# ruanjue/smartdenovo

Measured on AMD Instinct MI355X. Metric: Gbp of candidate pairs aligned/sec (wtzmo all-vs-all), higher is better.
Workload: dtype int32/int16

## Files before the change

### smartdenovo_amd/csrc/wtz_stitch_fused.h

```cpp
#ifndef WTZ_STITCH_FUSED_H
#define WTZ_STITCH_FUSED_H

#include "wtz_tasks.h"
#include "wtz_sw_frame.h"
#include "wtz_sw_frame16.h"

#ifdef __HIPCC__
template<int TW>
__device__ __attribute__((noinline)) bool wtz_extjob_run_fr_call(wtz_extjob_t *job, const wtz_params_t *Pm, wtz_pool_t *pool, wtz_pool_t *tpool){
	__shared__ uint64_t stb[TW];
	return wtz_extjob_run_fr<TW>(job, Pm, pool, tpool, stb);
}
template<int TW>
__device__ __attribute__((noinline)) void wtz_stitch_mid_call(uint32_t t, const wtz_env_t *V, const wtz_alnitem_t *items, wtz_stitch_state_t *sts, const wtz_extjob_t *jobsL, wtz_extjob_t *jobsR, const wtz_gapres_t *gaps){
	wtz_task_stitch_mid(t, *V, items, sts, jobsL, jobsR, gaps, true);
}
template<int TW>
__global__ void __launch_bounds__(64) __attribute__((amdgpu_waves_per_eu(WTZ_OCC_EXTFR, 8))) wtz_kernel_stitch_ext_fr(const wtz_env_t V, const wtz_alnitem_t *items, wtz_stitch_state_t *sts,
		wtz_extjob_t *jobsL, wtz_extjob_t *jobsR, const wtz_gapres_t *gaps, const uint32_t *order, uint32_t n, uint32_t stride, uint32_t first){
	const uint32_t b = blockIdx.x;
	if(b >= n) return;
	const uint32_t t = order[(size_t)b * stride + first];
	#pragma nounroll
	for(int side = 0; side < 2; side++){
		if(side){
			wtz_stitch_mid_call<TW>(t, &V, items, sts, jobsL, jobsR, gaps);
			__threadfence_block();
		}
		if(!wtz_extjob_run_fr_call<TW>(side ? &jobsR[t] : &jobsL[t], V.P, V.pool, V.pool + 1)) return;
		__threadfence_block();
	}
}
#define WTZ_PK_LDS_BYTES(TW) ((TW) * 8 + 64)
template<int TW>
__device__ __attribute__((always_inline)) inline bool wtz_extjob_run_pk_call(wtz_extjob_t *job, const wtz_params_t *Pm, wtz_pool_t *pool, wtz_pool_t *tpool){
	return wtz_extjob_run_pk<TW>(job, Pm, pool, tpool, (uint64_t*)wtz_wave_scratch());
}
template<int TW>
__global__ void __launch_bounds__(64) __attribute__((amdgpu_waves_per_eu(WTZ_OCC_EXTPK, 8))) wtz_kernel_stitch_ext_pk(const wtz_env_t V, const wtz_alnitem_t *items, wtz_stitch_state_t *sts,
		wtz_extjob_t *jobsL, wtz_extjob_t *jobsR, const wtz_gapres_t *gaps, const uint32_t *order, uint32_t n, uint32_t stride, uint32_t first, uint32_t *open){
	const uint32_t b = blockIdx.x;
	if(b >= n) return;
	const uint32_t t = order[(size_t)b * stride + first];
	#pragma nounroll
	for(int side = 0; side < 2; side++){
		if(side){
			wtz_task_stitch_mid(t, V, items, sts, jobsL, jobsR, gaps, true);
			__threadfence_block();
		}
		if(!wtz_extjob_run_pk_call<TW>(side ? &jobsR[t] : &jobsL[t], V.P, V.pool, V.pool + 1)){
			if((threadIdx.x & 63u) == 0){ const uint32_t k = atomicAdd(&open[0], 1u); open[1 + k] = t; }
			return;
		}
		__threadfence_block();
	}
}
#endif

#endif
```

### smartdenovo_amd/csrc/wtz_sw_frame16.h

```cpp
#ifndef WTZ_SW_FRAME16_H
#define WTZ_SW_FRAME16_H

#include "wtz_sw_frame.h"

#ifdef __HIPCC__

#ifndef WTZ_OCC_EXTPK
#define WTZ_OCC_EXTPK 4
#endif

typedef short wtz_v2s __attribute__((ext_vector_type(2)));
WTZ_D uint32_t wtz_pk_max(uint32_t a, uint32_t b){ return __builtin_bit_cast(uint32_t, __builtin_elementwise_max(__builtin_bit_cast(wtz_v2s, a), __builtin_bit_cast(wtz_v2s, b))); }
WTZ_D uint32_t wtz_pk_adds(uint32_t a, uint32_t b){ return __builtin_bit_cast(uint32_t, __builtin_elementwise_add_sat(__builtin_bit_cast(wtz_v2s, a), __builtin_bit_cast(wtz_v2s, b))); }
WTZ_D uint32_t wtz_pk_subs(uint32_t a, uint32_t b){ return __builtin_bit_cast(uint32_t, __builtin_elementwise_sub_sat(__builtin_bit_cast(wtz_v2s, a), __builtin_bit_cast(wtz_v2s, b))); }
WTZ_D uint32_t wtz_pk_mad(uint32_t a, uint32_t b, uint32_t c){ uint32_t r; asm("v_pk_mad_u16 %0, %1, %2, %3" : "=v"(r) : "v"(a), "v"(b), "v"(c)); return r; }
WTZ_D uint32_t wtz_bfi(uint32_t mask, uint32_t a, uint32_t b){ uint32_t r; asm("v_bfi_b32 %0, %1, %2, %3" : "=v"(r) : "s"(mask), "v"(a), "v"(b)); return r; }
WTZ_D uint32_t wtz_pk2(int32_t lo, int32_t hi){ return ((uint32_t)lo & 0xFFFFu) | ((uint32_t)hi << 16); }
WTZ_D int32_t wtz_pk_lo(uint32_t a){ return (int32_t)(int16_t)(a & 0xFFFFu); }
WTZ_D int32_t wtz_pk_hi(uint32_t a){ return (int32_t)a >> 16; }
WTZ_D uint32_t wtz_pk_join(uint32_t hi, uint32_t lo){ return __builtin_amdgcn_alignbit(hi, lo, 16); }
template<int H>
WTZ_D uint32_t wtz_pk_eqacc(uint32_t acc, uint32_t v, uint32_t t){
	if constexpr(H) asm("v_cmp_eq_u16_sdwa vcc, %1, %2 src0_sel:WORD_1 src1_sel:WORD_0\n\tv_addc_co_u32_e32 %0, vcc, %0, %0, vcc" : "+v"(acc) : "v"(v), "v"(t) : "vcc");
	else asm("v_cmp_eq_u16_sdwa vcc, %1, %2 src0_sel:WORD_0 src1_sel:WORD_0\n\tv_addc_co_u32_e32 %0, vcc, %0, %0, vcc" : "+v"(acc) : "v"(v), "v"(t) : "vcc");
	return acc;
}
WTZ_D uint32_t wtz_even_bits(uint64_t x){
	x &= 0x5555555555555555ULL;
	x = (x | (x >> 1)) & 0x3333333333333333ULL; x = (x | (x >> 2)) & 0x0F0F0F0F0F0F0F0FULL; x = (x | (x >> 4)) & 0x00FF00FF00FF00FFULL;
	x = (x | (x >> 8)) & 0x0000FFFF0000FFFFULL; x = (x | (x >> 16)) & 0x00000000FFFFFFFFULL;
	return (uint32_t)x;
}

template<int C2, int S>
WTZ_D void wtz_pk_row(uint32_t (&hv)[C2], uint32_t (&ev)[C2], uint32_t (&zw)[(C2 + 3) / 4], uint32_t (&gm)[(C2 + 3) / 4], const uint32_t eqw, const uint32_t bndp, const uint32_t SFp,
		const int32_t SF, const int32_t O, const uint32_t MXp, const uint32_t Xpp, const uint32_t Op, const uint32_t (&ckp)[C2]){
	uint32_t agg = 0x80008000u;
	auto cell1 = [&](auto kc, const uint32_t src) -> uint32_t {
		constexpr int k = decltype(kc)::value;
		const uint32_t b = (k ? (eqw >> k) : eqw) & 0x00010001u;
		const uint32_t m = wtz_pk_adds(wtz_pk_mad(b, MXp, src), Xpp);
		agg = wtz_pk_max(agg, m);
		return m;
	};
	if constexpr(S == 0){
		const uint32_t prv = (uint32_t)wtz_dpp_wave_shr1((int32_t)bndp, (int32_t)hv[C2 - 1]);
		const uint32_t src0 = wtz_pk_join(hv[C2 - 1], prv);
		wtz_static_for<0, C2>([&](auto kc){
			constexpr int k = C2 - 1 - decltype(kc)::value;
			hv[k] = cell1(wtz_ic<k>{}, (k == 0) ? src0 : hv[k == 0 ? 0 : k - 1]);
		});
	} else if constexpr(S == 1){
		wtz_static_for<0, C2>([&](auto kc){ constexpr int k = decltype(kc)::value; hv[k] = cell1(kc, hv[k]); });
	} else {
		const uint32_t nxt = (uint32_t)wtz_dpp_wave_shl1((int32_t)SFp, (int32_t)hv[0]);
		const uint32_t srcl = wtz_pk_join(nxt, hv[0]);
		wtz_static_for<0, C2>([&](auto kc){
			constexpr int k = decltype(kc)::value;
			hv[k] = cell1(kc, (k == C2 - 1) ? srcl : hv[k == C2 - 1 ? k : k + 1]);
		});
	}
	uint32_t f;
	{
		const int32_t aA = wtz_pk_lo(agg), aB = wtz_pk_hi(agg);
		const int32_t aL = aA > aB ? aA : aB;
		const int32_t pm = wtz_wave_max_scan_excl(aL + O, SF);
		const int32_t fA = pm > SF ? pm : SF;
		const int32_t fB = fA > aA + O ? fA : aA + O;
		f = wtz_pk2(fA, fB);
	}
	uint32_t ne0 = 0, ne1 = 0;
	if constexpr(S >= 1) ne0 = wtz_pk_join((uint32_t)wtz_dpp_wave_shl1((int32_t)SFp, (int32_t)ev[0]), ev[0]);
	if constexpr(S == 2) ne1 = wtz_pk_join((uint32_t)wtz_dpp_wave_shl1((int32_t)SFp, (int32_t)ev[C2 > 1 ? 1 : 0]), ev[C2 > 1 ? 1 : 0]);
	wtz_static_for<0, C2>([&](auto kc){
		constexpr int k = decltype(kc)::value;
		const uint32_t m = hv[k];
		uint32_t e;
		if constexpr(S == 0) e = ev[k];
		else if constexpr(S == 1) e = (k == C2 - 1) ? ne0 : ev[k == C2 - 1 ? k : k + 1];
		else e = (k == C2 - 1) ? ne1 : ((k == C2 - 2) ? ne0 : ev[k >= C2 - 2 ? k : k + 2]);
		const uint32_t h0 = wtz_pk_max(m, e);
		const uint32_t s0 = wtz_pk_subs(m, e);
		const uint32_t s1 = wtz_pk_subs(h0, f);
		const uint32_t h = wtz_pk_max(h0, f);
		const uint32_t t = wtz_pk_adds(m, Op);
		const uint32_t s2 = wtz_pk_subs(t, e);
		const uint32_t en = wtz_pk_max(e, t);
		const uint32_t s3 = wtz_pk_subs(t, f);
		f = wtz_pk_max(f, t);
		hv[k] = h; ev[k] = en;
		const uint32_t x01 = wtz_bfi(0x80008000u, s0, s1 >> 1), x23 = wtz_bfi(0x80008000u, s2, s3 >> 1);
		const uint32_t x = wtz_bfi(0xC000C000u, x01, x23 >> 2);
		const uint32_t v = wtz_pk_adds(h, ckp[k]);
		if constexpr((k & 3) == 0){ gm[k >> 2] = v; zw[k >> 2] = x >> 12; }
		else {
			gm[k >> 2] = wtz_pk_max(gm[k >> 2], v);
			if constexpr((k & 3) == 1) zw[k >> 2] = wtz_bfi(0x00F000F0u, x >> 8, zw[k >> 2]);
			else if constexpr((k & 3) == 2) zw[k >> 2] = wtz_bfi(0x0F000F00u, x >> 4, zw[k >> 2]);
			else zw[k >> 2] = wtz_bfi(0xF000F000u, x, zw[k >> 2]);
		}
		if constexpr((k & 3) == 3 || k == C2 - 1){ WTZ_PIN(zw[k >> 2]); }
	});
}

template<int C2>
WTZ_D bool wtz_shift_traceback_pk(wtz_aln_t &x, uint8_t **zchunk, const int32_t *zb, uint32_t zrow, uint32_t *lds, wtz_cigar_t &cigars, const wtz_tb_score *sc){
	const int lane = (int)(threadIdx.x & 63);
	constexpr int C = 2 * C2, CQ = (C2 + 3) / 4, NL = 64;
	constexpr int NLW = (128 / C) < NL ? (128 / C) : NL;
	constexpr int NDW = NLW * CQ, ROWB = NLW * C;
	static_assert(NDW <= 64 && ROWB <= 128, "window geometry");
	uint32_t *S32 = lds; uint8_t *S8 = (uint8_t*)lds; uint8_t *Sd = S8 + 8192;
	int32_t i_ = x.qe, j_ = x.te; uint32_t d_ = 0;
#ifdef WTZ_EXP_NOTB
	i_ = -1; j_ = -1;
#endif
	uint32_t run_op = 0xFFu, run_len = 0;
	int32_t n_gap_runs = 0; bool consistent = true;
	wtz_cigw_t Wr; Wr.v = &cigars; Wr.tail = 0;
	int32_t cc = 0;
	if(i_ >= 0) cc = j_ - wtz_as_global(zb)[i_];
	const int ln_off = lane / CQ, q4 = lane % CQ;
	while(i_ >= 0 && j_ >= 0){
		const int32_t i0 = i_;
		int32_t L0 = (cc < 0 ? 0 : (cc > NL * C - 1 ? NL * C - 1 : cc)) / C - NLW / 2;
		if(L0 > NL - NLW) L0 = NL - NLW;
		if(L0 < 0) L0 = 0;
		const int32_t CC0 = L0 * C;
		{
			const int32_t r = i0 - lane;
			Sd[lane] = (r >= 1) ? (uint8_t)(wtz_as_global(zb)[r] - wtz_as_global(zb)[r - 1]) : (uint8_t)0;
		}
		const int32_t cA = i0 >> 6;
		const uint8_t *chA = wtz_as_global(zchunk)[cA];
		const uint8_t *chB = cA > 0 ? wtz_as_global(zchunk)[cA - 1] : chA;
		const bool act = lane < NDW && (L0 + ln_off) < NL;
		const uint32_t doff = act ? ((uint32_t)q4 * (uint32_t)NL + (uint32_t)(L0 + ln_off)) * 4u : 0u;
		const uint32_t pos0 = (uint32_t)ln_off * (uint32_t)C + (uint32_t)q4 * 4u;
		for(int r8 = 0; r8 < 64; r8 += 8){
			uint32_t w8[8];
			#pragma unroll
			for(int u = 0; u < 8; u++){
				int32_t r = i0 - (r8 + u); if(r < 0) r = 0;
				const uint8_t *rowp = ((r >> 6) == cA ? chA : chB) + (size_t)(r & 63) * zrow;
				w8[u] = *wtz_as_global((const uint32_t*)(rowp + doff));
			}
			if(act){
				#pragma unroll
				for(int u = 0; u < 8; u++){
					const uint32_t pos = (uint32_t)(r8 + u) * 128u + pos0;
					#pragma unroll
					for(int hh = 0; hh < 2; hh++){
						uint32_t w = hh ? (w8[u] >> 16) : (w8[u] & 0xFFFFu);
						w = (w | (w << 8)) & 0x00FF00FFu; w = (w | (w << 4)) & 0x0F0F0F0Fu;
						const uint32_t a = (w >> 2) & 0x01010101u, b = (w >> 3) & 0x01010101u;
						const uint32_t v = (a << 1) | (b & (a ^ 0x01010101u)) | ((w & 0x02020202u) << 1) | ((w & 0x01010101u) << 5);
						const uint32_t p = pos + (hh ? (uint32_t)C2 : 0u);
						if constexpr((C2 & 3) == 0) S32[p >> 2] = v;
						else {
							#pragma unroll
							for(int k = 0; k < 4; k++) if(q4 * 4 + k < C2) S8[p + k] = (uint8_t)(v >> (8 * k));
						}
					}
				}
			}
		}
		__threadfence_block();
		if(lane == 0){
			while(i_ >= 0 && j_ >= 0){
				const int32_t rr = i0 - i_;
				if(rr >= 64) break;
				uint32_t zv = 0;
				if((uint32_t)cc < (uint32_t)(NL * C)){
					const int32_t t = cc - CC0;
					if((uint32_t)t >= (uint32_t)ROWB) break;
					zv = S8[rr * 128 + t];
				}
				const int32_t sft = (int32_t)Sd[rr];
				d_ = (zv >> (d_ << 1)) & 0x03;
				if(d_ == 0){ x.mat++; i_--; j_--; cc += sft - 1; }
				else if(d_ == 1){ i_--; x.ins++; cc += sft; }
				else { j_--; x.del++; cc--; }
				if(d_ == run_op) run_len++;
				else { if(run_len) wtz_cigw_push(Wr, run_op, run_len); run_op = d_; run_len = 1; if(d_) n_gap_runs++; }
			}
		}
		i_ = __builtin_amdgcn_readfirstlane(i_); j_ = __builtin_amdgcn_readfirstlane(j_); cc = __builtin_amdgcn_readfirstlane(cc);
		__threadfence_block();
	}
	if(lane == 0){
		if(run_len) wtz_cigw_push(Wr, run_op, run_len);
		if(i_ >= 0){ x.ins += i_ + 1; wtz_cigw_push(Wr, 1, (uint32_t)(i_ + 1)); n_gap_runs++; }
		if(j_ >= 0){ x.del += j_ + 1; wtz_cigw_push(Wr, 2, (uint32_t)(j_ + 1)); n_gap_runs++; }
		wtz_cigw_finish(Wr);
		wtz_cigar_reverse(cigars.a, cigars.n);
		const int32_t nd = x.mat, MXd = sc->M - sc->X;
		const long long S = (long long)x.score - sc->init - (long long)n_gap_runs * sc->O - (long long)sc->E * (x.ins + x.del) - (long long)sc->X * nd;
		if(MXd == 0 || S % MXd != 0 || S / MXd < 0 || S / MXd > nd) consistent = false;
		else { x.mat = (int32_t)(S / MXd); x.mis = nd - x.mat; }
		x.aln = x.mat + x.mis + x.ins + x.del; x.qe++; x.te++;
	}
	return __builtin_amdgcn_readfirstlane((int)consistent) != 0;
}

template<int C2, int TWD>
WTZ_D wtz_aln_t wtz_extend_shift_pk(int32_t qlen, const wtz_seq_packed &query, int32_t tlen, const wtz_seq_packed &target, int32_t init_score,
		int32_t ql, int32_t tl, int32_t W, int32_t M, int32_t X, int32_t O, int32_t E, int32_t T, int32_t bias, int32_t NG, int32_t SH,
		uint32_t *tp, wtz_trace_t &tr, wtz_pool_t *pool, wtz_cigar_t &cigars, unsigned long long *cells, bool *ok, bool *consistent){
	const int lane = (int)(threadIdx.x & 63);
	constexpr int C = 2 * C2, CQ = (C2 + 3) / 4;
	wtz_aln_t x; memset(&x, 0, sizeof x);
	*ok = true; *consistent = true;
	if(lane == 0) cigars.n = 0;
	if(init_score < 0) init_score = 0;
	qlen = __builtin_amdgcn_readfirstlane(qlen); tlen = __builtin_amdgcn_readfirstlane(tlen); init_score = __builtin_amdgcn_readfirstlane(init_score);
	ql = __builtin_amdgcn_readfirstlane(ql); tl = __builtin_amdgcn_readfirstlane(tl); W = __builtin_amdgcn_readfirstlane(W); bias = __builtin_amdgcn_readfirstlane(bias);
	NG = __builtin_amdgcn_readfirstlane(NG); SH = __builtin_amdgcn_readfirstlane(SH);
	M = __builtin_amdgcn_readfirstlane(M); X = __builtin_amdgcn_readfirstlane(X); O = __builtin_amdgcn_readfirstlane(O); E = __builtin_amdgcn_readfirstlane(E); T = __builtin_amdgcn_readfirstlane(T);
	const uint32_t zrow = (uint32_t)CQ * 256u;
	if(!wtz_trace_prepare(tr, pool, zrow, ql, true)){ *ok = false; return x; }
	uint8_t **zchunk = tr.chunk; int32_t *zb = tr.zb;
	uint8_t *z = NULL;
	{
		const int32_t nw = (tl + 31) / 32 + 2;
		for(int32_t w = lane; w < nw; w += 64){ const uint64_t pw = wtz_pack32(target, w * 32, tl); tp[w] = wtz_even_bits(pw); tp[TWD + w] = wtz_even_bits(pw >> 1); }
	}
	__threadfence_block();
	const int32_t colrel0 = lane * C;
	const int32_t MX = M - X, Xp = X - 2 * E;
	const uint32_t MXp = (uint32_t)__builtin_amdgcn_readfirstlane((int32_t)wtz_pk2(MX, MX)), Xpp = (uint32_t)__builtin_amdgcn_readfirstlane((int32_t)wtz_pk2(Xp, Xp)), Op = (uint32_t)__builtin_amdgcn_readfirstlane((int32_t)wtz_pk2(O, O));
	uint32_t ckp[C2];
	#pragma unroll
	for(int k = 0; k < C2; k++) ckp[k] = (uint32_t)__builtin_amdgcn_readfirstlane((int32_t)wtz_pk2(k * E, (C2 + k) * E));
	const int32_t lcE = colrel0 * E;
	uint32_t hv[C2], ev[C2];
	#pragma unroll
	for(int p = 0; p < C2; p++){
		int32_t vh[2], ve[2];
		#pragma unroll
		for(int hh = 0; hh < 2; hh++){
			const int32_t c = colrel0 + hh * C2 + p - 1;
			const int32_t hr = (c < 0) ? init_score : init_score + O + E * (c + 1);
			vh[hh] = hr - (c - 1) * E - bias;
			ve[hh] = NG - c * E - bias;
		}
		hv[p] = wtz_pk2(vh[0], vh[1]); ev[p] = wtz_pk2(ve[0], ve[1]);
	}
	int32_t mx = init_score, mi = -1, mj = -1, gmax = 0, gi = -1, gj = -1;
	int32_t jbp = -1, c = 0, i;
	unsigned long long ncell = 0;
	uint32_t qw_lo = 0, qw_hi = 0, qcur = 0;
	int32_t jb_n = 0, je_n = tl; uint32_t plo_n, phi_n;
	int32_t zbv = 0; bool lost = false;
	{
		if(je_n > W + 1) je_n = W + 1;
		if(je_n > tl) je_n = tl;
		const int32_t jj = colrel0 < tl ? colrel0 : (tl > 0 ? tl - 1 : 0);
		const int32_t w = jj >> 5; const uint32_t sh = (uint32_t)(jj & 31);
		plo_n = __builtin_amdgcn_alignbit(tp[w + 1], tp[w], sh); phi_n = __builtin_amdgcn_alignbit(tp[TWD + w + 1], tp[TWD + w], sh);
	}
	__builtin_amdgcn_s_waitcnt(0x0F70);
	for(i = 0; i < ql; i++){
		if((i & 63) == 0){
			const uint32_t ci = (uint32_t)i >> 6;
			unsigned long long za = 0;
			const int have = __builtin_amdgcn_readfirstlane(ci < tr.n_chunk ? 1 : 0);
			if(have) za = (unsigned long long)(uintptr_t)wtz_as_global(zchunk)[ci];
			else {
				if(lane == 0){ uint8_t *p = (uint8_t*)wtz_pool_alloc(pool, (size_t)zrow * 64); wtz_as_global(zchunk)[ci] = p; za = (unsigned long long)(uintptr_t)p; }
				za = __shfl(za, 0, 64);
			}
			const uint32_t zlo = (uint32_t)__builtin_amdgcn_readfirstlane((int)(uint32_t)za), zhi = (uint32_t)__builtin_amdgcn_readfirstlane((int)(uint32_t)(za >> 32));
			z = (uint8_t*)(uintptr_t)(((unsigned long long)zhi << 32) | zlo);
			if((zlo | zhi) == 0){ *ok = false; break; }
			if(!have) tr.n_chunk = ci + 1;
			if((i & 2047) == 0){ const uint64_t qw = wtz_pack32(query, i + lane * 32, ql); qw_lo = (uint32_t)qw; qw_hi = (uint32_t)(qw >> 32); }
			__builtin_amdgcn_s_waitcnt(0x0F70);
		}
		const int32_t jb = jb_n, je = je_n;
		if((i & 15) == 0){
			const int32_t qs = __builtin_amdgcn_readfirstlane((i & 2047) >> 5);
			qcur = (i & 16) ? (uint32_t)__builtin_amdgcn_readlane((int)qw_hi, qs) : (uint32_t)__builtin_amdgcn_readlane((int)qw_lo, qs);
		}
		const uint32_t qbase = (qcur >> ((i & 15) * 2)) & 3u;
		uint32_t eqw;
		{
			const uint32_t nl = (qbase & 1u) - 1u, nh = ((qbase >> 1) & 1u) - 1u;
			const uint32_t eq = (plo_n ^ nl) & (phi_n ^ nh);
			if constexpr(C2 == 16) eqw = eq;
			else eqw = (eq & ((1u << C2) - 1u)) | ((eq >> C2) << 16);
		}
		const int32_t s = __builtin_amdgcn_readfirstlane(jb - jbp);
		const int32_t bnd = ((jb == 0) ? init_score + O + E * i : NG) - (i + jb - 2) * E - bias;
		const int32_t SF = NG - (i + jb) * E - bias;
		const uint32_t bndp = (uint32_t)bnd << 16, SFp = wtz_pk2(SF, SF);
		uint32_t zw[CQ], gm[CQ];
		if(s == 1)      wtz_pk_row<C2, 1>(hv, ev, zw, gm, eqw, bndp, SFp, SF, O, MXp, Xpp, Op, ckp);
		else if(s == 0) wtz_pk_row<C2, 0>(hv, ev, zw, gm, eqw, bndp, SFp, SF, O, MXp, Xpp, Op, ckp);
		else            wtz_pk_row<C2, 2>(hv, ev, zw, gm, eqw, bndp, SFp, SF, O, MXp, Xpp, Op, ckp);
		const int32_t nvt = je - jb;
		const int32_t vcut = __builtin_amdgcn_readfirstlane(nvt / C2), kcut = __builtin_amdgcn_readfirstlane(nvt % C2);
		int32_t K;
		{
			uint32_t LM = gm[0];
			#pragma unroll
			for(int g = 1; g < CQ; g++) LM = wtz_pk_max(LM, gm[g]);
			if(kcut){
				uint32_t pm = 0x80008000u;
				wtz_uniform_switch<1, C2>(kcut, [&](auto kc){
					constexpr int KC = decltype(kc)::value, GF = KC / 4;
					uint32_t r = 0x80008000u;
					#pragma unroll
					for(int g = 0; g < GF; g++) r = wtz_pk_max(r, gm[g]);
					#pragma unroll
					for(int k = 4 * GF; k < KC; k++) r = wtz_pk_max(r, wtz_pk_adds(hv[k], ckp[k]));
					pm = r; WTZ_PIN_TAG(pm, KC);
				});
				const uint32_t hmask = (vcut & 1) ? 0xFFFF0000u : 0x0000FFFFu;
				const uint32_t LMc = (pm & hmask) | (LM & ~hmask);
				LM = (lane == (vcut >> 1)) ? LMc : LM;
			}
			const int32_t vA = wtz_pk_lo(LM) + lcE, vB = wtz_pk_hi(LM) + lcE;
			const int32_t kA = (colrel0 < nvt) ? (int32_t)(((uint32_t)vA << 7) + (uint32_t)(127 - 2 * lane)) : (int32_t)0x80000000;
			const int32_t kB = (colrel0 + C2 < nvt) ? (int32_t)(((uint32_t)vB << 7) + (uint32_t)(126 - 2 * lane)) : (int32_t)0x80000000;
			K = wtz_wave_max_i32(kA > kB ? kA : kB);
		}
		ncell += (unsigned long long)(je - jb);
		int32_t imax = 0, mj2 = -1;
		{
			const int32_t Hm = (K >> 7) + bias + (i + jb) * E;
			if(Hm > 0 && Hm > SH){
				imax = Hm;
				const int32_t vidx = 127 - (K & 127), Ls = vidx >> 1, hs = vidx & 1;
				const int32_t T16 = (K >> 7) - Ls * C * E;
				const int32_t klim = (vidx == vcut) ? kcut : C2;
				const uint32_t Tv = (uint32_t)T16 & 0xFFFFu;
				const int32_t nfull = klim >> 2;
				int32_t kf = -1;
				auto find = [&](auto hc){
					constexpr int H = decltype(hc)::value;
					uint32_t ag = 0;
					#pragma unroll
					for(int g = CQ - 1; g >= 0; g--) ag = wtz_pk_eqacc<H>(ag, gm[g], Tv);
					const uint32_t sg = (uint32_t)__builtin_amdgcn_readlane((int32_t)ag, Ls) & ((1u << nfull) - 1u);
					const int32_t gsel = sg ? (int32_t)__builtin_ctz(sg) : nfull;
					if(gsel < CQ){
						uint32_t ae = 0;
						wtz_uniform_switch<0, CQ>(gsel, [&](auto gc){
							constexpr int g = decltype(gc)::value;
							uint32_t a = 0;
							#pragma unroll
							for(int k = 4 * g + 3; k >= 4 * g; k--) a = (k < C2) ? wtz_pk_eqacc<H>(a, wtz_pk_adds(hv[k < C2 ? k : 0], ckp[k < C2 ? k : 0]), Tv) : a + a;
							ae = a; WTZ_PIN_TAG(ae, g);
						});
						const int32_t room = klim - 4 * gsel;
						const uint32_t se = (uint32_t)__builtin_amdgcn_readlane((int32_t)ae, Ls) & (room >= 4 ? 0xFu : ((1u << (room > 0 ? room : 0)) - 1u));
						if(se) kf = 4 * gsel + (int32_t)__builtin_ctz(se);
					}
				};
				if(hs) find(wtz_ic<1>{}); else find(wtz_ic<0>{});
				if(kf < 0){ lost = true; kf = 0; }
				mj2 = jb + Ls * C + hs * C2 + kf;
			}
		}
		zbv = (lane == (i & 63)) ? jb : zbv;
		if((i & 63) == 63) wtz_as_global(zb)[(i & ~63) + lane] = zbv;
		if(je == tlen){
			const int32_t idx = nvt - 1;
			const int32_t vr = __builtin_amdgcn_readfirstlane(idx / C2), kl = __builtin_amdgcn_readfirstlane(idx % C2);
			uint32_t hsel = 0;
			wtz_uniform_switch<0, C2>(kl, [&](auto kc){ constexpr int k = decltype(kc)::value; hsel = hv[k]; WTZ_PIN_TAG(hsel, k); });
			const uint32_t hw = (uint32_t)__builtin_amdgcn_readlane((int32_t)hsel, vr >> 1);
			const int32_t h1 = ((vr & 1) ? wtz_pk_hi(hw) : wtz_pk_lo(hw)) + bias + (i + je - 1) * E;
			if(h1 > SH && gmax < h1){ gmax = h1; gi = i; gj = je - 1; }
		}
		if(i + 1 == qlen && gmax < imax){ gmax = imax; gi = i; gj = mj2; }
		jbp = jb;
		bool stop = false;
		if(imax > mx){ mx = imax; mi = i; mj = mj2; }
		else if(imax <= 0) stop = true;
		if(!stop){
			c++; if(c < mj2) c++; else if(c > mj2) c--;
			jb_n = 0; je_n = tl;
			if(jb_n < c - W) jb_n = c - W;
			if(je_n > c + W + 1) je_n = c + W + 1;
			if(je_n > tl) je_n = tl;
			if(jb_n != jb){
				const int32_t j0n = jb_n + colrel0;
				const int32_t jj = j0n < tl ? j0n : (tl > 0 ? tl - 1 : 0);
				const int32_t w = jj >> 5; const uint32_t sh = (uint32_t)(jj & 31);
				plo_n = __builtin_amdgcn_alignbit(tp[w + 1], tp[w], sh); phi_n = __builtin_amdgcn_alignbit(tp[TWD + w + 1], tp[TWD + w], sh);
			}
			if(je_n > je){
				const int32_t SG = NG - (i + je) * E - bias, SE1 = NG - (i + 1 + je) * E - bias, SE2 = NG - (i + 2 + je) * E - bias;
				const uint32_t SGp = wtz_pk2(SG, SG), SE1p = wtz_pk2(SE1, SE1), SE2p = wtz_pk2(SE2, SE2);
				const int32_t Lb = vcut >> 1;
				const uint32_t hm1 = (vcut & 1) ? 0xFFFF0000u : 0x0000FFFFu;
				if(Lb < 64){
					wtz_uniform_switch<0, C2>(kcut, [&](auto kc){
						constexpr int k = decltype(kc)::value;
						const bool here = lane == Lb;
						hv[k] = here ? ((SGp & hm1) | (hv[k] & ~hm1)) : hv[k];
						ev[k] = here ? ((SE1p & hm1) | (ev[k] & ~hm1)) : ev[k];
						if constexpr(k + 1 < C2) ev[k + 1] = here ? ((SE2p & hm1) | (ev[k + 1] & ~hm1)) : ev[k + 1];
						else {
							const int32_t L2 = (vcut + 1) >> 1;
							ev[0] = (lane == L2) ? ((SE2p & ~hm1) | (ev[0] & hm1)) : ev[0];
						}
						WTZ_PIN_TAG(hv[k], k);
					});
				}
			}
		}
		if(colrel0 < nvt){
			WTZ_GLOBAL_AS uint32_t *zr = wtz_as_global((uint32_t*)(z + (size_t)(i & 63) * zrow) + lane);
			#pragma unroll
			for(int q4 = 0; q4 < CQ; q4++) zr[(size_t)q4 * 64] = zw[q4];
		}
		if(stop) break;
	}
	if(cells && lane == 0) *cells += ncell;
	if(!*ok) return x;
	{
		const int32_t last = i < ql ? i : ql - 1;
		if(last >= 0 && (last & 63) != 63 && lane <= (last & 63)) wtz_as_global(zb)[(last & ~63) + lane] = zbv;
	}
	if(gmax > 0 && gmax >= mx + T){ x.score = gmax; x.qe = gi; x.te = gj; }
	else { x.score = mx; x.qe = mi; x.te = mj; }
	__threadfence_block();
	const wtz_tb_score sc = { M, X, O, E, init_score };
	if(!wtz_shift_traceback_pk<C2>(x, zchunk, zb, zrow, tp, cigars, &sc)) *ok = false, *consistent = false;
	if(__builtin_amdgcn_readfirstlane((int)lost)) *ok = false, *consistent = false;
	return wtz_bcast_aln(x);
}

WTZ_D bool wtz_pk_window(const wtz_params_t *Pm, int32_t init_score, int32_t ql, int32_t tl, int32_t *bias, int32_t *ng, int32_t *sh){
	const long long M = Pm->M, X = Pm->X, O = Pm->O, E = Pm->E;
	if(E > 0 || E < -255 || X > 0 || M < 0 || O > 0 || M == X || M - X > 4096) return false;
	const long long aE = -E, aO = -O, aX = -X, Xp = X - 2 * E, Xm = Xp < 0 ? Xp : 0;
	const long long mn = ql < tl ? ql : tl;
	const long long hi = (long long)init_score + M * mn + ((long long)ql + tl + 4) * aE + (M - X) + 64;
	long long NG = -10000;
	long long lo = NG + ((long long)ql + 3) * Xm + O - 33 * aE - 64;
	*sh = -(1 << 30);
	if(hi - lo > 65000){
		if(M * mn >= 10000) return false;
		const long long step = aX > aO + aE ? aX : aO + aE;
		const long long Rlow = (long long)init_score - aO - ((long long)tl + 1) * aE - ((long long)ql + 1) * step - ((long long)ql + 2) * aO;
		NG = Rlow - M * mn - 64;
		if(NG <= -10000) return false;
		lo = NG - 33 * aE - 64;
		if(hi - lo > 65000) return false;
		*sh = (int32_t)(NG + M * mn);
	}
	*bias = (int32_t)((hi + lo) / 2); *ng = (int32_t)NG;
	return true;
}

WTZ_D bool wtz_pk_window_range(const wtz_params_t *Pm, int32_t ql, int32_t tl, long long i_lo, long long i_hi){
	const long long M = Pm->M, X = Pm->X, O = Pm->O, E = Pm->E;
	if(E > 0 || E < -255 || X > 0 || M < 0 || O > 0 || M == X || M - X > 4096) return false;
	if(i_lo < 0) i_lo = 0;
	if(i_hi < 0) i_hi = 0;
	const long long aE = -E, aO = -O, aX = -X, Xp = X - 2 * E, Xm = Xp < 0 ? Xp : 0;
	const long long mn = ql < tl ? ql : tl;
	const long long top = M * mn + ((long long)ql + tl + 4) * aE + (M - X) + 64;
	const long long lo_a = -10000 + ((long long)ql + 3) * Xm + O - 33 * aE - 64;
	const long long Ia = 65000 + lo_a - top;
	if(i_hi <= Ia) return true;
	if(M * mn >= 10000) return false;
	const long long step = aX > aO + aE ? aX : aO + aE;
	const long long fall = aO + ((long long)tl + 1) * aE + ((long long)ql + 1) * step + ((long long)ql + 2) * aO;
	const long long Ib = -10000 + 64 + M * mn + fall;
	const long long width_b = top + fall + M * mn + 64 + 33 * aE + 64;
	if(width_b > 65000) return false;
	return i_lo > Ib || Ib < Ia;
}

template<int TW>
WTZ_D bool wtz_extjob_run_pk(wtz_extjob_t *job, const wtz_params_t *Pm, wtz_pool_t *pool, wtz_pool_t *tpool, uint64_t *stb){
	if(!job->valid || job->done) return true;
	const int lane = (int)(threadIdx.x & 63);
	if(job->qlen <= 0 || job->tlen <= 0) return false;
	const int32_t init_score = job->init_score < 0 ? 0 : job->init_score;
	int32_t W = job->W, ql, tl, n_col;
	wtz_ext_geometry(job->qlen, job->tlen, init_score, W, Pm->M, Pm->O, Pm->O, Pm->E, Pm->T, ql, tl, n_col);
	const int32_t Cw = (n_col + 63) / 64;
	if(Cw > 32 || (tl + 31) / 32 + 3 > TW || (ql + 63) / 64 > WTZ_TRACE_MAXCHUNK) return false;
	int32_t bias = 0, ng = -10000, sh = 0;
	if(!wtz_pk_window(Pm, init_score, ql, tl, &bias, &ng, &sh)) return false;
	wtz_trace_t tr; tr.chunk = NULL; tr.zb = NULL; tr.n_chunk = 0; tr.zrow = 0; tr.cap_rows = 0;
	wtz_cigar_t cg; cg.a = NULL; cg.n = cg.cap = 0; cg.pool = pool; cg.bad = 0;
	if(lane == 0) cg.init(pool, (uint32_t)ql / 2u + 16u);
	unsigned long long cells = 0; bool ok = true, consistent = true;
	wtz_aln_t x;
#define WTZ_EXTPK_CASE(CM) x = wtz_extend_shift_pk<CM, TW>(job->qlen, job->q, job->tlen, job->t, job->init_score, ql, tl, W, Pm->M, Pm->X, Pm->O, Pm->E, Pm->T, bias, ng, sh, (uint32_t*)stb, tr, tpool, cg, &cells, &ok, &consistent)
	if(Cw <= 4) WTZ_EXTPK_CASE(2);
	else if(Cw <= 6) WTZ_EXTPK_CASE(3);
	else if(Cw <= 8) WTZ_EXTPK_CASE(4);
	else if(Cw <= 10) WTZ_EXTPK_CASE(5);
	else if(Cw <= 12) WTZ_EXTPK_CASE(6);
	else if(Cw <= 14) WTZ_EXTPK_CASE(7);
	else if(Cw <= 16) WTZ_EXTPK_CASE(8);
	else if(Cw <= 18) WTZ_EXTPK_CASE(9);
	else if(Cw <= 20) WTZ_EXTPK_CASE(10);
	else if(Cw <= 22) WTZ_EXTPK_CASE(11);
	else if(Cw <= 24) WTZ_EXTPK_CASE(12);
	else if(Cw <= 26) WTZ_EXTPK_CASE(13);
	else if(Cw <= 28) WTZ_EXTPK_CASE(14);
	else if(Cw <= 30) WTZ_EXTPK_CASE(15);
	else WTZ_EXTPK_CASE(16);
#undef WTZ_EXTPK_CASE
	if(!consistent) return false;
	if(lane == 0){ job->x = x; job->cigar = cg.a; job->cigar_len = cg.n; job->bad = (!ok || cg.bad); job->cells = cells; job->done = 7; }
	return true;
}

template<int TW>
__global__ void __launch_bounds__(64) __attribute__((amdgpu_waves_per_eu(WTZ_OCC_EXTPK, 8))) wtz_kernel_extjobs_pk(wtz_extjob_t *jobs, const uint32_t *order, uint32_t n, const wtz_params_t *Pm, wtz_pool_t *pool, wtz_pool_t *tpool){
	__shared__ uint64_t stb[TW];
	const uint32_t b = blockIdx.x;
	if(b >= n) return;
	(void)wtz_extjob_run_pk<TW>(&jobs[order ? order[b] : b], Pm, pool, tpool, stb);
}

#endif
#endif
```

Baseline: 10.73.

## Adapt packed-int16 band width per 64-row chunk during extension

The packed 16-bit banded extension kernel now picks its per-lane column count (C2) for each 64-row chunk from the current live band width, rather than fixing it per job from the maximum band. When the width changes, H/E state is relayed between lane layouts through an LDS relay buffer, and each trace chunk pointer records its width in the top byte so traceback can dispatch per chunk. This cuts wasted cell computation when the actual band is much narrower than the worst case. In exchange it adds relay overhead at each switch, more LDS use, more code through the uniform switch instantiations, and more register pressure from carry state.

```diff
diff --git a/smartdenovo_amd/csrc/wtz_stitch_fused.h b/smartdenovo_amd/csrc/wtz_stitch_fused.h
--- a/smartdenovo_amd/csrc/wtz_stitch_fused.h
+++ b/smartdenovo_amd/csrc/wtz_stitch_fused.h
@@ -31,7 +31,7 @@
 		__threadfence_block();
 	}
 }
-#define WTZ_PK_LDS_BYTES(TW) ((TW) * 8 + 64)
+#define WTZ_PK_LDS_BYTES(TW) ((TW) * 8 + 64 + WTZ_PK_RELAY_BYTES)
 template<int TW>
 __device__ __attribute__((always_inline)) inline bool wtz_extjob_run_pk_call(wtz_extjob_t *job, const wtz_params_t *Pm, wtz_pool_t *pool, wtz_pool_t *tpool){
 	return wtz_extjob_run_pk<TW>(job, Pm, pool, tpool, (uint64_t*)wtz_wave_scratch());
diff --git a/smartdenovo_amd/csrc/wtz_sw_frame16.h b/smartdenovo_amd/csrc/wtz_sw_frame16.h
--- a/smartdenovo_amd/csrc/wtz_sw_frame16.h
+++ b/smartdenovo_amd/csrc/wtz_sw_frame16.h
@@ -103,25 +103,71 @@
 	});
 }
 
+#ifndef WTZ_PK_CHUNK_WIDTH
+#define WTZ_PK_CHUNK_WIDTH 1
+#endif
+#define WTZ_PK_RELAY_COLS 384
+#define WTZ_PK_RELAY_BYTES (WTZ_PK_RELAY_COLS * 4)
+#define WTZ_PK_C2MAX 16
+#define WTZ_PK_CHUNK_ADDR(e) ((e) & 0x00FFFFFFFFFFFFFFull)
+#define WTZ_PK_CHUNK_C2(e) ((int32_t)((e) >> 56))
+
+WTZ_D int32_t wtz_pk_chunk_c2(const int32_t nvt_now, const int32_t c2j){
+#if WTZ_PK_CHUNK_WIDTH
+	int32_t c = (nvt_now + 130 + 127) >> 7;
+	if(c < 2) c = 2;
+	return 4 * c <= 3 * c2j ? c : c2j;
+#else
+	(void)nvt_now; return c2j;
+#endif
+}
+
 template<int C2>
-WTZ_D bool wtz_shift_traceback_pk(wtz_aln_t &x, uint8_t **zchunk, const int32_t *zb, uint32_t zrow, uint32_t *lds, wtz_cigar_t &cigars, const wtz_tb_score *sc){
+WTZ_D void wtz_pk_relay_put(const uint32_t (&h)[WTZ_PK_C2MAX], const uint32_t (&e)[WTZ_PK_C2MAX], uint16_t *rl, const int32_t P0, const int32_t P1){
+	const int32_t base = (int32_t)(threadIdx.x & 63) * 2 * C2;
+	#pragma unroll
+	for(int k = 0; k < C2; k++){
+		#pragma unroll
+		for(int hh = 0; hh < 2; hh++){
+			const int32_t p = base + hh * C2 + k;
+			if(p >= P0 && p < P1){
+				rl[p - P0] = (uint16_t)(hh ? (h[k] >> 16) : h[k]);
+				rl[WTZ_PK_RELAY_COLS + p - P0] = (uint16_t)(hh ? (e[k] >> 16) : e[k]);
+			}
+		}
+	}
+}
+template<int C2>
+WTZ_D void wtz_pk_relay_get(uint32_t (&h)[WTZ_PK_C2MAX], uint32_t (&e)[WTZ_PK_C2MAX], const uint16_t *rl, const int32_t P0, const int32_t P1){
+	const int32_t base = (int32_t)(threadIdx.x & 63) * 2 * C2;
+	#pragma unroll
+	for(int k = 0; k < C2; k++){
+		#pragma unroll
+		for(int hh = 0; hh < 2; hh++){
+			const int32_t p = base + hh * C2 + k;
+			if(p >= P0 && p < P1){
+				const uint32_t vh = rl[p - P0], ve = rl[WTZ_PK_RELAY_COLS + p - P0];
+				h[k] = hh ? ((h[k] & 0x0000FFFFu) | (vh << 16)) : ((h[k] & 0xFFFF0000u) | vh);
+				e[k] = hh ? ((e[k] & 0x0000FFFFu) | (ve << 16)) : ((e[k] & 0xFFFF0000u) | ve);
+			}
+		}
+	}
+}
+
+typedef struct { int32_t i_, j_, cc; uint32_t d_, run_op, run_len; int32_t n_gap_runs; wtz_cigw_t Wr; } wtz_pk_walk_t;
+
+template<int C2>
+WTZ_D void wtz_pk_tb_window(wtz_pk_walk_t &s, wtz_aln_t &x, const uint8_t *chA, const uint8_t *chB, const int32_t nrow, const int32_t *zb, uint32_t *lds){
 	const int lane = (int)(threadIdx.x & 63);
 	constexpr int C = 2 * C2, CQ = (C2 + 3) / 4, NL = 64;
+	constexpr uint32_t zrow = (uint32_t)CQ * 256u;
 	constexpr int NLW = (128 / C) < NL ? (128 / C) : NL;
 	constexpr int NDW = NLW * CQ, ROWB = NLW * C;
 	static_assert(NDW <= 64 && ROWB <= 128, "window geometry");
 	uint32_t *S32 = lds; uint8_t *S8 = (uint8_t*)lds; uint8_t *Sd = S8 + 8192;
-	int32_t i_ = x.qe, j_ = x.te; uint32_t d_ = 0;
-#ifdef WTZ_EXP_NOTB
-	i_ = -1; j_ = -1;
-#endif
-	uint32_t run_op = 0xFFu, run_len = 0;
-	int32_t n_gap_runs = 0; bool consistent = true;
-	wtz_cigw_t Wr; Wr.v = &cigars; Wr.tail = 0;
-	int32_t cc = 0;
-	if(i_ >= 0) cc = j_ - wtz_as_global(zb)[i_];
+	int32_t i_ = s.i_, j_ = s.j_, cc = s.cc; uint32_t d_ = s.d_;
 	const int ln_off = lane / CQ, q4 = lane % CQ;
-	while(i_ >= 0 && j_ >= 0){
+	{
 		const int32_t i0 = i_;
 		int32_t L0 = (cc < 0 ? 0 : (cc > NL * C - 1 ? NL * C - 1 : cc)) / C - NLW / 2;
 		if(L0 > NL - NLW) L0 = NL - NLW;
@@ -132,8 +178,6 @@
 			Sd[lane] = (r >= 1) ? (uint8_t)(wtz_as_global(zb)[r] - wtz_as_global(zb)[r - 1]) : (uint8_t)0;
 		}
 		const int32_t cA = i0 >> 6;
-		const uint8_t *chA = wtz_as_global(zchunk)[cA];
-		const uint8_t *chB = cA > 0 ? wtz_as_global(zchunk)[cA - 1] : chA;
 		const bool act = lane < NDW && (L0 + ln_off) < NL;
 		const uint32_t doff = act ? ((uint32_t)q4 * (uint32_t)NL + (uint32_t)(L0 + ln_off)) * 4u : 0u;
 		const uint32_t pos0 = (uint32_t)ln_off * (uint32_t)C + (uint32_t)q4 * 4u;
@@ -169,7 +213,7 @@
 		if(lane == 0){
 			while(i_ >= 0 && j_ >= 0){
 				const int32_t rr = i0 - i_;
-				if(rr >= 64) break;
+				if(rr >= nrow) break;
 				uint32_t zv = 0;
 				if((uint32_t)cc < (uint32_t)(NL * C)){
 					const int32_t t = cc - CC0;
@@ -181,21 +225,45 @@
 				if(d_ == 0){ x.mat++; i_--; j_--; cc += sft - 1; }
 				else if(d_ == 1){ i_--; x.ins++; cc += sft; }
 				else { j_--; x.del++; cc--; }
-				if(d_ == run_op) run_len++;
-				else { if(run_len) wtz_cigw_push(Wr, run_op, run_len); run_op = d_; run_len = 1; if(d_) n_gap_runs++; }
+				if(d_ == s.run_op) s.run_len++;
+				else { if(s.run_len) wtz_cigw_push(s.Wr, s.run_op, s.run_len); s.run_op = d_; s.run_len = 1; if(d_) s.n_gap_runs++; }
 			}
 		}
 		i_ = __builtin_amdgcn_readfirstlane(i_); j_ = __builtin_amdgcn_readfirstlane(j_); cc = __builtin_amdgcn_readfirstlane(cc);
 		__threadfence_block();
 	}
+	s.i_ = i_; s.j_ = j_; s.cc = cc; s.d_ = d_;
+}
+
+WTZ_D bool wtz_shift_traceback_pk(wtz_aln_t &x, uint8_t **zchunk, const int32_t *zb, uint32_t *lds, wtz_cigar_t &cigars, const wtz_tb_score *sc){
+	const int lane = (int)(threadIdx.x & 63);
+	wtz_pk_walk_t s;
+	s.i_ = x.qe; s.j_ = x.te; s.d_ = 0;
+#ifdef WTZ_EXP_NOTB
+	s.i_ = -1; s.j_ = -1;
+#endif
+	s.run_op = 0xFFu; s.run_len = 0; s.n_gap_runs = 0; bool consistent = true;
+	s.Wr.v = &cigars; s.Wr.tail = 0;
+	s.cc = 0;
+	if(s.i_ >= 0) s.cc = s.j_ - wtz_as_global(zb)[s.i_];
+	const unsigned long long *ze = (const unsigned long long*)zchunk;
+	while(s.i_ >= 0 && s.j_ >= 0){
+		const int32_t cA = s.i_ >> 6;
+		const unsigned long long eA = wtz_as_global(ze)[cA], eB = cA > 0 ? wtz_as_global(ze)[cA - 1] : eA;
+		const int32_t wA = __builtin_amdgcn_readfirstlane(WTZ_PK_CHUNK_C2(eA)), wB = __builtin_amdgcn_readfirstlane(WTZ_PK_CHUNK_C2(eB));
+		const uint8_t *chA = (const uint8_t*)(uintptr_t)WTZ_PK_CHUNK_ADDR(eA);
+		const uint8_t *chB = (wA == wB) ? (const uint8_t*)(uintptr_t)WTZ_PK_CHUNK_ADDR(eB) : chA;
+		const int32_t nrow = (wA == wB) ? 64 : (s.i_ & 63) + 1;
+		wtz_uniform_switch<2, WTZ_PK_C2MAX + 1>(wA, [&](auto wc){ wtz_pk_tb_window<decltype(wc)::value>(s, x, chA, chB, nrow, zb, lds); });
+	}
 	if(lane == 0){
-		if(run_len) wtz_cigw_push(Wr, run_op, run_len);
-		if(i_ >= 0){ x.ins += i_ + 1; wtz_cigw_push(Wr, 1, (uint32_t)(i_ + 1)); n_gap_runs++; }
-		if(j_ >= 0){ x.del += j_ + 1; wtz_cigw_push(Wr, 2, (uint32_t)(j_ + 1)); n_gap_runs++; }
-		wtz_cigw_finish(Wr);
+		if(s.run_len) wtz_cigw_push(s.Wr, s.run_op, s.run_len);
+		if(s.i_ >= 0){ x.ins += s.i_ + 1; wtz_cigw_push(s.Wr, 1, (uint32_t)(s.i_ + 1)); s.n_gap_runs++; }
+		if(s.j_ >= 0){ x.del += s.j_ + 1; wtz_cigw_push(s.Wr, 2, (uint32_t)(s.j_ + 1)); s.n_gap_runs++; }
+		wtz_cigw_finish(s.Wr);
 		wtz_cigar_reverse(cigars.a, cigars.n);
 		const int32_t nd = x.mat, MXd = sc->M - sc->X;
-		const long long S = (long long)x.score - sc->init - (long long)n_gap_runs * sc->O - (long long)sc->E * (x.ins + x.del) - (long long)sc->X * nd;
+		const long long S = (long long)x.score - sc->init - (long long)s.n_gap_runs * sc->O - (long long)sc->E * (x.ins + x.del) - (long long)sc->X * nd;
 		if(MXd == 0 || S % MXd != 0 || S / MXd < 0 || S / MXd > nd) consistent = false;
 		else { x.mat = (int32_t)(S / MXd); x.mis = nd - x.mat; }
 		x.aln = x.mat + x.mis + x.ins + x.del; x.qe++; x.te++;
@@ -203,76 +271,78 @@
 	return __builtin_amdgcn_readfirstlane((int)consistent) != 0;
 }
 
+typedef struct {
+	int32_t mx, mi, mj, gmax, gi, gj;
+	int32_t jbp, jep, c, i, jb_n, je_n;
+	int32_t zbv; uint32_t qw_lo, qw_hi, qcur;
+	unsigned long long ncell;
+	bool lost, stop, fail;
+} wtz_pk_carry_t;
+typedef struct { int32_t qlen, tlen, init_score, ql, tl, W, M, X, O, E, T, bias, NG, SH, C2J; uint32_t zrowJ; } wtz_pk_job_t;
+
 template<int C2, int TWD>
-WTZ_D wtz_aln_t wtz_extend_shift_pk(int32_t qlen, const wtz_seq_packed &query, int32_t tlen, const wtz_seq_packed &target, int32_t init_score,
-		int32_t ql, int32_t tl, int32_t W, int32_t M, int32_t X, int32_t O, int32_t E, int32_t T, int32_t bias, int32_t NG, int32_t SH,
-		uint32_t *tp, wtz_trace_t &tr, wtz_pool_t *pool, wtz_cigar_t &cigars, unsigned long long *cells, bool *ok, bool *consistent){
+WTZ_D void wtz_pk_rows(const wtz_pk_job_t &J, wtz_pk_carry_t &S, uint32_t (&hS)[WTZ_PK_C2MAX], uint32_t (&eS)[WTZ_PK_C2MAX], const wtz_seq_packed &query,
+		const uint32_t *tp, wtz_trace_t &tr, wtz_pool_t *pool){
 	const int lane = (int)(threadIdx.x & 63);
 	constexpr int C = 2 * C2, CQ = (C2 + 3) / 4;
-	wtz_aln_t x; memset(&x, 0, sizeof x);
-	*ok = true; *consistent = true;
-	if(lane == 0) cigars.n = 0;
-	if(init_score < 0) init_score = 0;
-	qlen = __builtin_amdgcn_readfirstlane(qlen); tlen = __builtin_amdgcn_readfirstlane(tlen); init_score = __builtin_amdgcn_readfirstlane(init_score);
-	ql = __builtin_amdgcn_readfirstlane(ql); tl = __builtin_amdgcn_readfirstlane(tl); W = __builtin_amdgcn_readfirstlane(W); bias = __builtin_amdgcn_readfirstlane(bias);
-	NG = __builtin_amdgcn_readfirstlane(NG); SH = __builtin_amdgcn_readfirstlane(SH);
-	M = __builtin_amdgcn_readfirstlane(M); X = __builtin_amdgcn_readfirstlane(X); O = __builtin_amdgcn_readfirstlane(O); E = __builtin_amdgcn_readfirstlane(E); T = __builtin_amdgcn_readfirstlane(T);
-	const uint32_t zrow = (uint32_t)CQ * 256u;
-	if(!wtz_trace_prepare(tr, pool, zrow, ql, true)){ *ok = false; return x; }
+	constexpr uint32_t zrow = (uint32_t)CQ * 256u;
+	const int32_t qlen = J.qlen, tlen = J.tlen, init_score = J.init_score, ql = J.ql, tl = J.tl, W = J.W, O = J.O, E = J.E, bias = J.bias, NG = J.NG, SH = J.SH;
 	uint8_t **zchunk = tr.chunk; int32_t *zb = tr.zb;
 	uint8_t *z = NULL;
-	{
-		const int32_t nw = (tl + 31) / 32 + 2;
-		for(int32_t w = lane; w < nw; w += 64){ const uint64_t pw = wtz_pack32(target, w * 32, tl); tp[w] = wtz_even_bits(pw); tp[TWD + w] = wtz_even_bits(pw >> 1); }
-	}
-	__threadfence_block();
 	const int32_t colrel0 = lane * C;
-	const int32_t MX = M - X, Xp = X - 2 * E;
+	const int32_t MX = J.M - J.X, Xp = J.X - 2 * E;
 	const uint32_t MXp = (uint32_t)__builtin_amdgcn_readfirstlane((int32_t)wtz_pk2(MX, MX)), Xpp = (uint32_t)__builtin_amdgcn_readfirstlane((int32_t)wtz_pk2(Xp, Xp)), Op = (uint32_t)__builtin_amdgcn_readfirstlane((int32_t)wtz_pk2(O, O));
 	uint32_t ckp[C2];
 	#pragma unroll
 	for(int k = 0; k < C2; k++) ckp[k] = (uint32_t)__builtin_amdgcn_readfirstlane((int32_t)wtz_pk2(k * E, (C2 + k) * E));
 	const int32_t lcE = colrel0 * E;
 	uint32_t hv[C2], ev[C2];
-	#pragma unroll
-	for(int p = 0; p < C2; p++){
-		int32_t vh[2], ve[2];
+	if(S.i == 0){
 		#pragma unroll
-		for(int hh = 0; hh < 2; hh++){
-			const int32_t c = colrel0 + hh * C2 + p - 1;
-			const int32_t hr = (c < 0) ? init_score : init_score + O + E * (c + 1);
-			vh[hh] = hr - (c - 1) * E - bias;
-			ve[hh] = NG - c * E - bias;
-		}
-		hv[p] = wtz_pk2(vh[0], vh[1]); ev[p] = wtz_pk2(ve[0], ve[1]);
-	}
-	int32_t mx = init_score, mi = -1, mj = -1, gmax = 0, gi = -1, gj = -1;
-	int32_t jbp = -1, c = 0, i;
-	unsigned long long ncell = 0;
-	uint32_t qw_lo = 0, qw_hi = 0, qcur = 0;
-	int32_t jb_n = 0, je_n = tl; uint32_t plo_n, phi_n;
-	int32_t zbv = 0; bool lost = false;
+		for(int p = 0; p < C2; p++){
+			int32_t vh[2], ve[2];
+			#pragma unroll
+			for(int hh = 0; hh < 2; hh++){
+				const int32_t c = colrel0 + hh * C2 + p - 1;
+				const int32_t hr = (c < 0) ? init_score : init_score + O + E * (c + 1);
+				vh[hh] = hr - (c - 1) * E - bias;
+				ve[hh] = NG - c * E - bias;
+			}
+			hv[p] = wtz_pk2(vh[0], vh[1]); ev[p] = wtz_pk2(ve[0], ve[1]);
+		}
+	} else {
+		#pragma unroll
+		for(int p = 0; p < C2; p++){ hv[p] = hS[p]; ev[p] = eS[p]; }
+	}
+	int32_t mx = S.mx, mi = S.mi, mj = S.mj, gmax = S.gmax, gi = S.gi, gj = S.gj;
+	int32_t jbp = S.jbp, jep = S.jep, c = S.c, i = S.i;
+	unsigned long long ncell = S.ncell;
+	uint32_t qw_lo = S.qw_lo, qw_hi = S.qw_hi, qcur = S.qcur;
+	int32_t jb_n = S.jb_n, je_n = S.je_n; uint32_t plo_n, phi_n;
+	int32_t zbv = S.zbv; bool lost = S.lost;
 	{
-		if(je_n > W + 1) je_n = W + 1;
-		if(je_n > tl) je_n = tl;
-		const int32_t jj = colrel0 < tl ? colrel0 : (tl > 0 ? tl - 1 : 0);
+		const int32_t j0n = jb_n + colrel0;
+		const int32_t jj = j0n < tl ? j0n : (tl > 0 ? tl - 1 : 0);
 		const int32_t w = jj >> 5; const uint32_t sh = (uint32_t)(jj & 31);
 		plo_n = __builtin_amdgcn_alignbit(tp[w + 1], tp[w], sh); phi_n = __builtin_amdgcn_alignbit(tp[TWD + w + 1], tp[TWD + w], sh);
 	}
+	const int32_t i_in = i;
 	__builtin_amdgcn_s_waitcnt(0x0F70);
-	for(i = 0; i < ql; i++){
+	for(; i < ql; i++){
 		if((i & 63) == 0){
+			if(i != i_in && wtz_pk_chunk_c2(je_n - jb_n, J.C2J) != C2) break;
 			const uint32_t ci = (uint32_t)i >> 6;
 			unsigned long long za = 0;
 			const int have = __builtin_amdgcn_readfirstlane(ci < tr.n_chunk ? 1 : 0);
-			if(have) za = (unsigned long long)(uintptr_t)wtz_as_global(zchunk)[ci];
-			else {
-				if(lane == 0){ uint8_t *p = (uint8_t*)wtz_pool_alloc(pool, (size_t)zrow * 64); wtz_as_global(zchunk)[ci] = p; za = (unsigned long long)(uintptr_t)p; }
-				za = __shfl(za, 0, 64);
-			}
+			if(lane == 0){
+				uint8_t *p = have ? (uint8_t*)(uintptr_t)WTZ_PK_CHUNK_ADDR(wtz_as_global((unsigned long long*)zchunk)[ci]) : (uint8_t*)wtz_pool_alloc(pool, (size_t)J.zrowJ * 64);
+				za = (unsigned long long)(uintptr_t)p;
+				wtz_as_global((unsigned long long*)zchunk)[ci] = p ? (za | ((unsigned long long)C2 << 56)) : 0ull;
+			}
+			za = __shfl(za, 0, 64);
 			const uint32_t zlo = (uint32_t)__builtin_amdgcn_readfirstlane((int)(uint32_t)za), zhi = (uint32_t)__builtin_amdgcn_readfirstlane((int)(uint32_t)(za >> 32));
 			z = (uint8_t*)(uintptr_t)(((unsigned long long)zhi << 32) | zlo);
-			if((zlo | zhi) == 0){ *ok = false; break; }
+			if((zlo | zhi) == 0){ S.fail = true; break; }
 			if(!have) tr.n_chunk = ci + 1;
 			if((i & 2047) == 0){ const uint64_t qw = wtz_pack32(query, i + lane * 32, ql); qw_lo = (uint32_t)qw; qw_hi = (uint32_t)(qw >> 32); }
 			__builtin_amdgcn_s_waitcnt(0x0F70);
@@ -375,7 +445,7 @@
 			if(h1 > SH && gmax < h1){ gmax = h1; gi = i; gj = je - 1; }
 		}
 		if(i + 1 == qlen && gmax < imax){ gmax = imax; gi = i; gj = mj2; }
-		jbp = jb;
+		jbp = jb; jep = je;
 		bool stop = false;
 		if(imax > mx){ mx = imax; mi = i; mj = mj2; }
 		else if(imax <= 0) stop = true;
@@ -417,20 +487,85 @@
 			#pragma unroll
 			for(int q4 = 0; q4 < CQ; q4++) zr[(size_t)q4 * 64] = zw[q4];
 		}
-		if(stop) break;
-	}
-	if(cells && lane == 0) *cells += ncell;
-	if(!*ok) return x;
+		if(stop){ S.stop = true; break; }
+	}
+	#pragma unroll
+	for(int p = 0; p < WTZ_PK_C2MAX; p++){ hS[p] = p < C2 ? hv[p < C2 ? p : 0] : 0u; eS[p] = p < C2 ? ev[p < C2 ? p : 0] : 0u; }
+	S.mx = mx; S.mi = mi; S.mj = mj; S.gmax = gmax; S.gi = gi; S.gj = gj;
+	S.jbp = jbp; S.jep = jep; S.c = c; S.i = i; S.jb_n = jb_n; S.je_n = je_n;
+	S.zbv = zbv; S.qw_lo = qw_lo; S.qw_hi = qw_hi; S.qcur = qcur; S.ncell = ncell; S.lost = lost;
+}
+
+template<int TWD>
+WTZ_D wtz_aln_t wtz_extend_shift_pk(int32_t C2J, int32_t qlen, const wtz_seq_packed &query, int32_t tlen, const wtz_seq_packed &target, int32_t init_score,
+		int32_t ql, int32_t tl, int32_t W, int32_t M, int32_t X, int32_t O, int32_t E, int32_t T, int32_t bias, int32_t NG, int32_t SH,
+		uint32_t *tp, wtz_trace_t &tr, wtz_pool_t *pool, wtz_cigar_t &cigars, unsigned long long *cells, bool *ok, bool *consistent){
+	const int lane = (int)(threadIdx.x & 63);
+	wtz_aln_t x; memset(&x, 0, sizeof x);
+	*ok = true; *consistent = true;
+	if(lane == 0) cigars.n = 0;
+	if(init_score < 0) init_score = 0;
+	wtz_pk_job_t J;
+	J.C2J = __builtin_amdgcn_readfirstlane(C2J);
+	J.qlen = __builtin_amdgcn_readfirstlane(qlen); J.tlen = __builtin_amdgcn_readfirstlane(tlen); J.init_score = __builtin_amdgcn_readfirstlane(init_score);
+	J.ql = ql = __builtin_amdgcn_readfirstlane(ql); J.tl = tl = __builtin_amdgcn_readfirstlane(tl); J.W = W = __builtin_amdgcn_readfirstlane(W); J.bias = __builtin_amdgcn_readfirstlane(bias);
+	J.NG = __builtin_amdgcn_readfirstlane(NG); J.SH = __builtin_amdgcn_readfirstlane(SH);
+	J.M = __builtin_amdgcn_readfirstlane(M); J.X = __builtin_amdgcn_readfirstlane(X); J.O = __builtin_amdgcn_readfirstlane(O); J.E = __builtin_amdgcn_readfirstlane(E); J.T = __builtin_amdgcn_readfirstlane(T);
+	J.zrowJ = (uint32_t)((J.C2J + 3) / 4) * 256u;
+	if(!wtz_trace_prepare(tr, pool, J.zrowJ, ql, true)){ *ok = false; return x; }
 	{
-		const int32_t last = i < ql ? i : ql - 1;
-		if(last >= 0 && (last & 63) != 63 && lane <= (last & 63)) wtz_as_global(zb)[(last & ~63) + lane] = zbv;
-	}
-	if(gmax > 0 && gmax >= mx + T){ x.score = gmax; x.qe = gi; x.te = gj; }
-	else { x.score = mx; x.qe = mi; x.te = mj; }
+		const int32_t nw = (tl + 31) / 32 + 2;
+		for(int32_t w = lane; w < nw; w += 64){ const uint64_t pw = wtz_pack32(target, w * 32, tl); tp[w] = wtz_even_bits(pw); tp[TWD + w] = wtz_even_bits(pw >> 1); }
+	}
 	__threadfence_block();
-	const wtz_tb_score sc = { M, X, O, E, init_score };
-	if(!wtz_shift_traceback_pk<C2>(x, zchunk, zb, zrow, tp, cigars, &sc)) *ok = false, *consistent = false;
-	if(__builtin_amdgcn_readfirstlane((int)lost)) *ok = false, *consistent = false;
+	uint16_t *rl = (uint16_t*)(tp + 2 * TWD);
+	wtz_pk_carry_t S;
+	S.mx = J.init_score; S.mi = -1; S.mj = -1; S.gmax = 0; S.gi = -1; S.gj = -1;
+	S.jbp = -1; S.jep = -1; S.c = 0; S.i = 0; S.ncell = 0; S.qw_lo = 0; S.qw_hi = 0; S.qcur = 0; S.zbv = 0;
+	S.lost = false; S.stop = false; S.fail = false;
+	S.jb_n = 0; S.je_n = tl;
+	if(S.je_n > W + 1) S.je_n = W + 1;
+	if(S.je_n > tl) S.je_n = tl;
+	uint32_t hS[WTZ_PK_C2MAX], eS[WTZ_PK_C2MAX];
+	#pragma unroll
+	for(int k = 0; k < WTZ_PK_C2MAX; k++){ hS[k] = 0; eS[k] = 0; }
+	int32_t c2cur = 0;
+	while(S.i < ql && !S.stop && !S.fail){
+		const int32_t c2n = __builtin_amdgcn_readfirstlane(wtz_pk_chunk_c2(S.je_n - S.jb_n, J.C2J));
+		if(S.i > 0 && c2n != c2cur){
+			int32_t nT = S.jep - S.jbp + 2;
+			if(nT > 128 * c2cur) nT = 128 * c2cur;
+			if(nT > 128 * c2n) nT = 128 * c2n;
+			const int32_t SG = J.NG - (S.i - 1 + S.jep) * J.E - J.bias;
+			const uint32_t SGp = wtz_pk2(SG, SG);
+			uint32_t hN[WTZ_PK_C2MAX], eN[WTZ_PK_C2MAX];
+			#pragma unroll
+			for(int k = 0; k < WTZ_PK_C2MAX; k++){ hN[k] = SGp; eN[k] = SGp; }
+			for(int32_t P0 = 0; P0 < nT; P0 += WTZ_PK_RELAY_COLS){
+				const int32_t P1 = P0 + WTZ_PK_RELAY_COLS < nT ? P0 + WTZ_PK_RELAY_COLS : nT;
+				wtz_uniform_switch<2, WTZ_PK_C2MAX + 1>(c2cur, [&](auto wc){ wtz_pk_relay_put<decltype(wc)::value>(hS, eS, rl, P0, P1); });
+				__threadfence_block();
+				wtz_uniform_switch<2, WTZ_PK_C2MAX + 1>(c2n, [&](auto wc){ wtz_pk_relay_get<decltype(wc)::value>(hN, eN, rl, P0, P1); });
+				__threadfence_block();
+			}
+			#pragma unroll
+			for(int k = 0; k < WTZ_PK_C2MAX; k++){ hS[k] = hN[k]; eS[k] = eN[k]; }
+		}
+		c2cur = c2n;
+		wtz_uniform_switch<2, WTZ_PK_C2MAX + 1>(c2n, [&](auto wc){ wtz_pk_rows<decltype(wc)::value, TWD>(J, S, hS, eS, query, tp, tr, pool); });
+	}
+	if(cells && lane == 0) *cells += S.ncell;
+	if(S.fail){ *ok = false; return x; }
+	{
+		const int32_t last = S.i < ql ? S.i : ql - 1;
+		if(last >= 0 && (last & 63) != 63 && lane <= (last & 63)) wtz_as_global(tr.zb)[(last & ~63) + lane] = S.zbv;
+	}
+	if(S.gmax > 0 && S.gmax >= S.mx + J.T){ x.score = S.gmax; x.qe = S.gi; x.te = S.gj; }
+	else { x.score = S.mx; x.qe = S.mi; x.te = S.mj; }
+	__threadfence_block();
+	const wtz_tb_score sc = { J.M, J.X, J.O, J.E, J.init_score };
+	if(!wtz_shift_traceback_pk(x, tr.chunk, tr.zb, tp, cigars, &sc)) *ok = false, *consistent = false;
+	if(__builtin_amdgcn_readfirstlane((int)S.lost)) *ok = false, *consistent = false;
 	return wtz_bcast_aln(x);
 }
 
@@ -494,23 +629,8 @@
 	if(lane == 0) cg.init(pool, (uint32_t)ql / 2u + 16u);
 	unsigned long long cells = 0; bool ok = true, consistent = true;
 	wtz_aln_t x;
-#define WTZ_EXTPK_CASE(CM) x = wtz_extend_shift_pk<CM, TW>(job->qlen, job->q, job->tlen, job->t, job->init_score, ql, tl, W, Pm->M, Pm->X, Pm->O, Pm->E, Pm->T, bias, ng, sh, (uint32_t*)stb, tr, tpool, cg, &cells, &ok, &consistent)
-	if(Cw <= 4) WTZ_EXTPK_CASE(2);
-	else if(Cw <= 6) WTZ_EXTPK_CASE(3);
-	else if(Cw <= 8) WTZ_EXTPK_CASE(4);
-	else if(Cw <= 10) WTZ_EXTPK_CASE(5);
-	else if(Cw <= 12) WTZ_EXTPK_CASE(6);
-	else if(Cw <= 14) WTZ_EXTPK_CASE(7);
-	else if(Cw <= 16) WTZ_EXTPK_CASE(8);
-	else if(Cw <= 18) WTZ_EXTPK_CASE(9);
-	else if(Cw <= 20) WTZ_EXTPK_CASE(10);
-	else if(Cw <= 22) WTZ_EXTPK_CASE(11);
-	else if(Cw <= 24) WTZ_EXTPK_CASE(12);
-	else if(Cw <= 26) WTZ_EXTPK_CASE(13);
-	else if(Cw <= 28) WTZ_EXTPK_CASE(14);
-	else if(Cw <= 30) WTZ_EXTPK_CASE(15);
-	else WTZ_EXTPK_CASE(16);
-#undef WTZ_EXTPK_CASE
+	const int32_t C2J = Cw <= 4 ? 2 : (Cw + 1) / 2;
+	x = wtz_extend_shift_pk<TW>(C2J, job->qlen, job->q, job->tlen, job->t, job->init_score, ql, tl, W, Pm->M, Pm->X, Pm->O, Pm->E, Pm->T, bias, ng, sh, (uint32_t*)stb, tr, tpool, cg, &cells, &ok, &consistent);
 	if(!consistent) return false;
 	if(lane == 0){ job->x = x; job->cigar = cg.a; job->cigar_len = cg.n; job->bad = (!ok || cg.bad); job->cells = cells; job->done = 7; }
 	return true;
@@ -518,7 +638,7 @@
 
 template<int TW>
 __global__ void __launch_bounds__(64) __attribute__((amdgpu_waves_per_eu(WTZ_OCC_EXTPK, 8))) wtz_kernel_extjobs_pk(wtz_extjob_t *jobs, const uint32_t *order, uint32_t n, const wtz_params_t *Pm, wtz_pool_t *pool, wtz_pool_t *tpool){
-	__shared__ uint64_t stb[TW];
+	__shared__ uint64_t stb[TW + WTZ_PK_RELAY_BYTES / 8];
 	const uint32_t b = blockIdx.x;
 	if(b >= n) return;
 	(void)wtz_extjob_run_pk<TW>(&jobs[order ? order[b] : b], Pm, pool, tpool, stb);
```

New measurement: 10.56. 1.6% lower.
